# jameshball/kidney-diffusion

Hardware: AMD Instinct MI355X
Metric: denoising-steps/sec (64->256 SR UNet, bs16) (higher is better)
Workload: dtype f32

## Files before the change

include/kd_engine.h:

```cpp
#ifndef KD_ENGINE_H
#define KD_ENGINE_H

#include <stddef.h>
#include <stdint.h>

#ifdef __cplusplus
extern "C" {
#endif

#define KD_MAX_LEVELS 8

const char* kd_last_error(void);
#define KD_ENGINE_ABI_VERSION 2
int kd_version(void);
const char* kd_build_id(void);

typedef struct kd_unet_config {
  int dim;
  int num_levels;
  int dim_mults[KD_MAX_LEVELS];
  int num_resnet_blocks[KD_MAX_LEVELS];
  int layer_attns[KD_MAX_LEVELS];
  int layer_cross_attns[KD_MAX_LEVELS];
  int cond_dim;
// ... 214 lines not shown
int kd_conv3x3_winograd_nhwc(const float* d_x, const float* d_w_oihw, const float* d_bias, float* d_y,
                             int B, int H, int W, int Cin, int Cout, void* stream);
int kd_conv3x3_winograd4_nhwc(const float* d_x, const float* d_w_oihw, const float* d_bias, const float* d_res,
                              float* d_y, int B, int H, int W, int Cin, int Cout, int G, float eps,
                              float* d_out_stats, int gemm_bf16x3, void* stream);
int kd_gemm_bf16x3(const float* d_a, const float* d_b, float* d_c, int G, int M, int N, int K, int a_planes, void* stream);
int kd_linear_bf16x3(const float* d_x, int ldx, const float* d_w, const float* d_bias, const float* d_res, int ldres,
                     const float* d_gate_src, int ldgs, const float* d_gate, int hw, float* d_y, int ldy, int M, int N, int K,
                     int act, int pixshuf_wo, double* d_seg, void* stream);
int kd_linear_bf16x3_seg_rows(int M, int N, int K);
int kd_downsample_bf16x3(const float* d_x, int ldx, const float* d_w, const float* d_bias, float* d_y, int B, int H, int W, int C,
                         int O, double* d_seg, void* stream);
int kd_gn_conv3x3_winograd_fused_nhwc(const float* d_x, const float* d_gamma, const float* d_beta,
                                      const float* d_scale_shift, const float* d_w_oihw,
                                      const float* d_bias, const float* d_res, float* d_y, int B, int H,
                                      int W, int Cin, int Cout, int G, float eps, float* d_out_stats,
                                      int ldx, void* stream);

int kd_linear_skinny(const float* d_x, int ldx, const float* d_w, const float* d_bias, float* d_y, int ldy, int M, int K,
                     int N, int in_act, int act, void* stream);
int kd_global_context_gate(const float* d_x, int B, int HW, int C, const float* d_wk, const float* d_bk, const float* d_w0,
                           const float* d_b0, int hid, const float* d_w2, const float* d_b2, float* d_gate, float* d_pooled,
                           int path, void* stream);
int kd_gate_add_nhwc(const float* d_a, const float* d_gate, const float* d_r, int ldr, float* d_y, int ldy, double* d_seg,
                     int B, int HW, int C, void* stream);
int kd_gate_add_chunks(int B, int HW);
int kd_linattn_chunk_tokens(void);
int kd_linattn_dwconv_nhwc(const float* d_x, const float* d_wq, const float* d_wk, const float* d_wv, float* d_y,
                           float* d_part, int B, int H, int W, int heads, void* stream);
int kd_linattn_context(const float* d_k, const float* d_v, int ld, const float* d_part, int HW, const float* d_ck,
                       const float* d_cv, int ldc, int m, const float* d_null_k, const float* d_null_v, float* d_ctx, int B,
                       int heads, void* stream);
int kd_linattn_apply(const float* d_q, int ldq, const float* d_ctx, float* d_out, int ldo, int B, int N, int heads,
                     float scale, int silu, void* stream);
int kd_gn_fold_seg(const double* d_seg0, int nseg0, int nchunk0, float scale0, float ab_mul0, const double* d_seg1, int nseg1,
                   int nchunk1, float scale1, float ab_mul1, const float* d_gamma, const float* d_beta,
                   const float* d_scale_shift, int ld_ss, float* d_ab, float* d_stats, int B, int HW, int C, int G, float eps,
                   void* stream);
float kd_wf_ab_scale(void);
int kd_gn_conv3x3_winograd4_nhwc(const float* d_x, int ldx, const float* d_stats, const float* d_gamma, const float* d_beta,
                                 const float* d_scale_shift, int ld_ss, int skip_c0, float skip_scale, const float* d_w_oihw,
                                 const float* d_bias, const float* d_res, int ldres, float* d_y, double* d_out_seg, int B,
                                 int H, int W, int Cin, int Cout, int G, int gemm_mode, int images_per_set, void* stream);

int kd_init_conv_nchw(const float* d_x, const float* d_w3, const float* d_w7, const float* d_w15,
                      const float* d_bias, float* d_y, int B, int S, int n3, int n7, int n15, void* stream);
// ... 59 lines not shown
```

kidney-diffusion_amd/csrc/api.inc:

```
extern "C" {

const char* kd_last_error(void) { return kd::g_err.c_str(); }
int kd_version(void) { return KD_ENGINE_ABI_VERSION; }

int kd_unet_create(const kd_unet_config_t* cfg, const kd_param_t* params, int n_params, kd_unet_t** out) {
  return kd_unet_create_shared(cfg, params, n_params, nullptr, out);
}

int kd_unet_create_shared(const kd_unet_config_t* cfg, const kd_param_t* params, int n_params,
                          const kd_unet_t* share_with, kd_unet_t** out) {
  return kd_unet_create_self_cond(cfg, params, n_params, share_with, 0, out);
}

int kd_unet_create_self_cond(const kd_unet_config_t* cfg, const kd_param_t* params, int n_params,
                             const kd_unet_t* share_with, int self_cond, kd_unet_t** out) {
  kd_unet_ext_t ext;
  memset(&ext, 0, sizeof ext);
  ext.self_cond = self_cond;
  return kd_unet_create_ext(cfg, params, n_params, share_with, &ext, out);
}

int kd_unet_create_ext(const kd_unet_config_t* cfg, const kd_param_t* params, int n_params, const kd_unet_t* share_with,
                       const kd_unet_ext_t* ext, kd_unet_t** out) {
  return kd_unet_create_ext2(cfg, params, n_params, share_with, ext, nullptr, out);
// ... 680 lines not shown
}

int kd_linattn_apply(const float* d_q, int ldq, const float* d_ctx, float* d_out, int ldo, int B, int N, int heads,
                     float scale, int silu, void* stream) {
  hipStream_t s = (hipStream_t)stream;
  KD_REQUIRE(d_q && d_ctx && d_out, "kd_linattn_apply: null argument");
  return entry_finish(launch_linattn_apply(d_q, ldq, d_ctx, d_out, ldo, B, N, heads, scale, silu, s), s);
}

int kd_global_context_gate(const float* d_x, int B, int HW, int C, const float* d_wk, const float* d_bk, const float* d_w0,
                           const float* d_b0, int hid, const float* d_w2, const float* d_b2, float* d_gate, float* d_pooled,
                           int path, void* stream) {
  hipStream_t s = (hipStream_t)stream;
  KD_REQUIRE(d_x && d_wk && d_bk && d_w0 && d_b0 && d_w2 && d_b2 && d_gate, "kd_global_context_gate: null argument");
  KD_REQUIRE(B > 0 && HW > 0 && hid > 0 && C % 4 == 0 && C > 0 && C <= 2048,
             "kd_global_context_gate needs B, HW, hid > 0 and C % 4 == 0, C <= 2048");
  KD_REQUIRE(path >= 0 && path <= 2, "kd_global_context_gate: path 0 (the plan's choice), 1 (pool + two linears), 2 (fused)");
  const bool fused_ok = gca_gate_fused_ok(C, hid) && (((uintptr_t)d_w0 | (uintptr_t)d_w2) & 15) == 0;
  KD_REQUIRE(path != 2 || fused_ok, "kd_global_context_gate: the fused gate needs C <= 512, hid <= 256, 16-byte aligned weights");
  const bool fused = path == 2 || (path == 0 && gca_gate_fused_ok(C, hid) && B > 1);
  KD_REQUIRE(!(fused && d_pooled), "kd_global_context_gate: the fused gate does not leave the pooled vector");
  EntryBufs bufs;
  float *scratch = nullptr, *pooled = d_pooled, *hidden = nullptr;
  if (bufs.get((void**)&scratch, gca_scratch_floats(B, HW, C) * sizeof(float))) return 1;
  if (fused) return entry_finish(launch_gca_gate(d_x, d_wk, d_bk, scratch, d_w0, d_b0, hid, d_w2, d_b2, d_gate, B, HW, C, s), s);
  if (!pooled && bufs.get((void**)&pooled, (size_t)B * C * sizeof(float))) return 1;
  if (bufs.get((void**)&hidden, (size_t)B * hid * sizeof(float))) return 1;
  int rc = launch_gca_pool(d_x, d_wk, d_bk, nullptr, pooled, scratch, B, HW, C, s);
  if (!rc) rc = launch_linear_skinny(pooled, C, d_w0, d_b0, hidden, hid, B, C, hid, ACT_NONE, ACT_SILU, s);
  if (!rc) rc = launch_linear_skinny(hidden, hid, d_w2, d_b2, d_gate, C, B, hid, C, ACT_NONE, ACT_SIGMOID, s);
  return entry_finish(rc, s);
}

int kd_gate_add_chunks(int B, int HW) { return B > 0 && HW > 0 ? gate_add_chunks(B, HW) : 0; }

int kd_gate_add_nhwc(const float* d_a, const float* d_gate, const float* d_r, int ldr, float* d_y, int ldy, double* d_seg,
                     int B, int HW, int C, void* stream) {
  hipStream_t s = (hipStream_t)stream;
  if (ldr <= 0) ldr = C;
  if (ldy <= 0) ldy = C;
  KD_REQUIRE(d_a && d_r && d_y, "kd_gate_add_nhwc: null argument");
  KD_REQUIRE(B > 0 && HW > 0 && C > 0 && C % 4 == 0 && ldr >= C && ldy >= C && ldr % 4 == 0 && ldy % 4 == 0,
             "kd_gate_add_nhwc needs C % 4 == 0 and row strides >= C, multiples of 4");
  KD_REQUIRE((((uintptr_t)d_a | (uintptr_t)d_gate | (uintptr_t)d_r | (uintptr_t)d_y) & 15) == 0,
             "kd_gate_add_nhwc: 16-byte aligned maps and gate");
  KD_REQUIRE(!d_seg || C % 16 == 0, "kd_gate_add_nhwc: segment partials need C % 16 == 0");
  return entry_finish(launch_gate_add(d_a, d_gate, d_r, ldr, d_y, ldy, d_seg, B, HW, C, s), s);
}

float kd_wf_ab_scale(void) { return WF_AB_SCALE; }

int kd_gn_fold_seg(const double* d_seg0, int nseg0, int nchunk0, float scale0, float ab_mul0, const double* d_seg1, int nseg1,
                   int nchunk1, float scale1, float ab_mul1, const float* d_gamma, const float* d_beta,
                   const float* d_scale_shift, int ld_ss, float* d_ab, float* d_stats, int B, int HW, int C, int G, float eps,
// ... 389 lines not shown
```

kidney-diffusion_amd/csrc/common.h:

```cpp
#pragma once
#include <hip/hip_runtime.h>
#include <stdint.h>
#include <stdio.h>
#include <algorithm>
#include <string>

#ifdef KD_EXPERIMENT
#include "../../scratch/experiment_switch.h"
#else
constexpr int kd_switch(const char*, int dflt) { return dflt; }
#endif

namespace kd {

void set_error(const std::string& msg);

#define KD_HIP_CHECK(expr)                                                               \
  do {                                                                                   \
    hipError_t _e = (expr);                                                              \
    if (_e != hipSuccess) {                                                              \
      ::kd::set_error(std::string(#expr) + " failed: " + hipGetErrorString(_e) + " at " + \
                      __FILE__ + ":" + std::to_string(__LINE__));                        \
      return 1;                                                                          \
    }                                                                                    \
// ... 160 lines not shown
int launch_copy_rows(const float* src, int64_t src_bstride, int ld_src, float* dst, int64_t dst_bstride,
                     int ld_dst, int rows, int C, int B, hipStream_t s);
int launch_bcast_row(const float* src, float* dst, int64_t dst_bstride, int C, int B, hipStream_t s);

struct KVSeg {
  const float* k;
  const float* v;
  int ld;
  int n;
};
int launch_attention(const float* q, int ldq, const float* null_k, const float* null_v, KVSeg s0, KVSeg s1,
                     float* out, int ldo, int B, int Nq, int H, int Hkv, int D, float scale, hipStream_t s);
int attention_key_tile(int D);
int launch_linear_gemv(const float* x, const float* w, const float* bias, float* y, int K, int N, int in_act, int act,
                       hipStream_t s);
int launch_linear_skinny(const float* x, int ldx, const float* w, const float* bias, float* y, int ldy, int M,
                         int K, int N, int in_act, int act, hipStream_t s);
int launch_linear_skinny_valu(const float* x, int ldx, const float* w, const float* bias, float* y, int ldy, int M,
                              int K, int N, int in_act, int act, hipStream_t s);
int launch_gca_pool(const float* x, const float* wk, const float* bk, float* logits, float* pooled,
                    float* scratch, int B, int HW, int C, hipStream_t s);
size_t gca_scratch_floats(int B, int HW, int C);
bool gca_gate_fused_ok(int C, int hid);
int launch_gca_gate(const float* x, const float* wk, const float* bk, float* scratch, const float* w0, const float* b0, int hid,
                    const float* w2, const float* b2, float* gate, int B, int HW, int C, hipStream_t s);
int launch_sinu_emb(const float* t, const float* w, float* out, int B, int half, hipStream_t s);

bool init_conv_fused_ok(int S, int n3, int n7, int n15, int np);
size_t init_conv_weight_floats(int n3, int n7, int n15, int np);
int launch_init_conv_pack(const float* w3, const float* w7, const float* w15, float* out, int n3, int n7, int n15, int Itot,
                          int c0, int np, hipStream_t s);
int launch_init_conv(const float* x_nchw, const float* sc_nchw, int cx, int np, const float* wp, const float* bias, const float* res,
                     float* y, int ldy, double* seg, int B, int S, int n3, int n7, int n15, hipStream_t s);
bool init_plain_ok(int S, int n, int k, int np);
size_t init_plain_weight_floats(int n, int k, int np);
int launch_init_plain_pack(const float* w_oihw, float* out, int n, int Itot, int c0, int np, int k, hipStream_t s);
int launch_init_plain(const float* x_nchw, const float* sc_nchw, int cx, int np, const float* wp, const float* bias, const float* res,
                      float* y, int ldy, double* seg, int B, int S, int n, int k, hipStream_t s);

constexpr int LA_CHUNK = 64;
int linattn_chunks(int HW);
int linattn_splits(int B, int heads, int HW);
size_t linattn_ws_floats(int B, int heads, int HW);
int launch_linattn_pack_dw(const float* wq, const float* wk, const float* wv, float* dst, int inner, hipStream_t s);
int launch_linattn_dwconv(const float* x, const float* w, float* y, float* part, int B, int H, int W, int inner,
                          hipStream_t s);
// ... 97 lines not shown
```

kidney-diffusion_amd/csrc/engine.hip:

```cpp
#include <stdlib.h>
#include <string.h>

#include <algorithm>
#include <cstddef>
#include <functional>
#include <map>
#include <memory>
#include <stdexcept>
#include <string>
#include <type_traits>
#include <unordered_map>
#include <unordered_set>
#include <vector>

#include "../../include/kd_engine.h"
#include "common.h"

namespace kd {

static thread_local std::string g_err;
void set_error(const std::string& msg) { g_err = msg; }

#define KD_THROW_IF(expr)                                          \
  do {                                                             \
// ... 988 lines not shown
    free(proj);
    T h1 = linear(h0, P(f + ".1.weight", (int64_t)hidden * dim), nullptr, hidden, gelu_late ? ACT_NONE : ACT_GELU);
    free(h0);
    T h2 = layernorm(h1, P(f + ".3.g", hidden), nullptr, nullptr, gelu_late ? ACT_GELU : ACT_NONE, nullptr, nullptr, false,
                     linear_is_x3(h1, dim, &x1, dst) ? 1 : 0);
    free(h1);
    T y = linear(h2, P(f + ".4.weight", (int64_t)dim * hidden), nullptr, dim, ACT_NONE, &x1, dst);
    free(h2);
    free(x1);
    return y;
  }

  T gca(const T& h, const std::string& pre) {
    int C = h.C, hid = std::max(3, C / 2);
    const float* wk = P(pre + ".to_k.weight", C);
    const float* bk = P(pre + ".to_k.bias", 1);
    const float* w0 = P(pre + ".net.0.weight", (int64_t)hid * C);
    const float* b0 = P(pre + ".net.0.bias", hid);
    const float* w2 = P(pre + ".net.2.weight", (int64_t)C * hid);
    const float* b2 = P(pre + ".net.2.bias", C);
    int Bx = h.B, HW = h.HW();
    const Ref hr = at(h);
    if (gca_gate_fused_ok(C, hid) && h.B > 1 && kd_switch("KD_GCA_FUSED", 1)) {
      T scratch = alloc_bytes(gca_scratch_floats(h.B, h.HW(), C) * sizeof(float));
      T gate = alloc(h.B, 1, 1, C);
      const Ref sr = at(scratch), gr = at(gate);
      emit([=](hipStream_t s) {
        return launch_gca_gate(hr.f(), wk, bk, sr.f(), w0, b0, hid, w2, b2, gr.f(), Bx, HW, C, s);
      }, "gca_gate HW" + std::to_string(HW) + " C" + std::to_string(C));
      u->macs += (int64_t)Bx * HW * C * 2 + (int64_t)Bx * C * hid * 2;
      free(scratch);
      return gate;
    }
    T logits = alloc(h.B, h.H, h.W, 1);
    T pooled = alloc(h.B, 1, 1, C);
    T scratch = alloc_bytes(gca_scratch_floats(h.B, h.HW(), C) * sizeof(float));
    const Ref lr = at(logits), pr = at(pooled), sr = at(scratch);
    emit([=](hipStream_t s) {
      return launch_gca_pool(hr.f(), wk, bk, lr.f(), pr.f(), sr.f(), Bx, HW, C, s);
    }, "gca_pool HW" + std::to_string(HW) + " C" + std::to_string(C));
    u->macs += (int64_t)Bx * HW * C * 2;
    free(logits);
    free(scratch);
    T hidden = alloc(h.B, 1, 1, hid);
    skinny(at(pooled), C, w0, b0, at(hidden), hid, h.B, C, hid, ACT_NONE, ACT_SILU);
    free(pooled);
    T gate = alloc(h.B, 1, 1, C);
// ... 610 lines not shown
```

kidney-diffusion_amd/csrc/kernels_small.hip:

```cpp
#include "common.h"

namespace kd {

typedef float f32x16 __attribute__((ext_vector_type(16)));
typedef float f32x4 __attribute__((ext_vector_type(4)));

__device__ __forceinline__ float act_s(float v, int act) {
  if (act == ACT_SILU) return v / (1.0f + expf(-v));
  if (act == ACT_GELU) return 0.5f * v * (1.0f + erff(v * 0.70710678118654752440f));
  if (act == ACT_SIGMOID) return 1.0f / (1.0f + expf(-v));
  return v;
}
__device__ __forceinline__ float wave_sum(float v) {
#pragma unroll
  for (int off = 32; off > 0; off >>= 1) v += __shfl_xor(v, off, 64);
  return v;
}

constexpr int SKM_UNROLL = 8;

template <int KW>
__global__ __launch_bounds__(64 * KW) void linear_skinny_mfma_kernel(const float* __restrict__ x, int ldx,
                                                                    const float* __restrict__ w,
                                                                    const float* __restrict__ bias,
// ... 73 lines not shown
  KD_REQUIRE(M > 0 && N > 0 && K > 0, "skinny linear: empty");
  const bool mfma_ok = (K & 3) == 0 && (ldx & 3) == 0 && (((uintptr_t)x) & 15) == 0 && (((uintptr_t)w) & 15) == 0;
  if (!mfma_ok) return launch_linear_skinny_valu(x, ldx, w, bias, y, ldy, M, K, N, in_act, act, s);
  if (M == 1 && K <= 16384) return launch_linear_gemv(x, w, bias, y, K, N, in_act, act, s);
  dim3 grid((N + 31) / 32, (M + 31) / 32);
  if (K >= 512)
    hipLaunchKernelGGL(linear_skinny_mfma_kernel<4>, grid, dim3(256), 0, s, x, ldx, w, bias, y, ldy, M, K, N, in_act, act);
  else
    hipLaunchKernelGGL(linear_skinny_mfma_kernel<1>, grid, dim3(64), 0, s, x, ldx, w, bias, y, ldy, M, K, N, in_act, act);
  KD_HIP_CHECK(hipGetLastError());
  return 0;
}

constexpr int GCA_ROWS = 256;
static inline int gca_rows(int HW, int B) {
  int r = GCA_ROWS;
  while ((HW + r - 1) / r > 1024) r *= 2;
  while (r > 32 && (int64_t)((HW + r - 1) / r) * B < 1024 && (HW + r / 2 - 1) / (r / 2) <= 1024) r /= 2;
  return r;
}
constexpr int GCA_MAXT = 8;
constexpr int GCA_U = 4;

template <int T, int RPW>
__global__ __launch_bounds__(256) void gca_partial_kernel(const float* __restrict__ x, const float* __restrict__ wk,
                                                          const float* __restrict__ bk, float* __restrict__ part,
                                                          int HW, int C, int rows) {
  extern __shared__ float sm[];
  const int b = blockIdx.y, chunk = blockIdx.x, nchunks = gridDim.x;
  const int lane = threadIdx.x & 63, wave = threadIdx.x >> 6;
  constexpr int LPR = 64 / RPW;
  const int sub = RPW == 2 ? (lane >> 5) : 0;
  const int li = RPW == 2 ? (lane & 31) : lane;
  const int C4 = C >> 2;
  const int p0 = chunk * rows, p1 = min(HW, p0 + rows);
  f32x4 wv[T], acc[T];
  const f32x4 z = {0.f, 0.f, 0.f, 0.f};
#pragma unroll
  for (int t = 0; t < T; ++t) {
    int c4 = li + LPR * t;
    wv[t] = c4 < C4 ? *(const f32x4*)(wk + c4 * 4) : z;
    acc[t] = z;
  }
  const float bias = bk[0];
  float mrun = -INFINITY, lrun = 0.f;
  const int stride = 4 * RPW;
  for (int pb = p0 + wave * RPW + sub; pb < p1; pb += stride * GCA_U) {
    f32x4 xv[GCA_U][T];
#pragma unroll
    for (int u = 0; u < GCA_U; ++u) {
// ... 39 lines not shown
    mrun = mn;
  }
  float* sacc = sm;
  float* sml = sm + 4 * C;
  if (lane == 0) {
    sml[wave * 2] = mrun;
    sml[wave * 2 + 1] = lrun;
  }
  if (sub == 0) {
#pragma unroll
    for (int t = 0; t < T; ++t) {
      int c4 = li + LPR * t;
      if (c4 < C4) *(f32x4*)(sacc + wave * C + c4 * 4) = acc[t];
    }
  }
  __syncthreads();
  float mb = fmaxf(fmaxf(sml[0], sml[2]), fmaxf(sml[4], sml[6]));
  float sc[4], lb = 0.f;
#pragma unroll
  for (int wv_ = 0; wv_ < 4; ++wv_) {
    sc[wv_] = sml[wv_ * 2] == -INFINITY ? 0.f : expf(sml[wv_ * 2] - mb);
    lb += sml[wv_ * 2 + 1] * sc[wv_];
  }
  float* out = part + ((int64_t)b * nchunks + chunk) * (C + 2);
  for (int c = threadIdx.x; c < C; c += 256)
    out[2 + c] = (sacc[c] * sc[0] + sacc[C + c] * sc[1]) + (sacc[2 * C + c] * sc[2] + sacc[3 * C + c] * sc[3]);
  if (threadIdx.x == 0) {
    out[0] = mb;
    out[1] = lb;
  }
}

__global__ __launch_bounds__(256) void gca_combine_kernel(const float* __restrict__ part, float* __restrict__ pooled,
                                                          int nchunks, int C) {
  __shared__ float se[1024];
  __shared__ float red[8];
  __shared__ float sacc[16][16];
  const int b = blockIdx.x, lane = threadIdx.x & 63, wave = threadIdx.x >> 6;
  const int cl = threadIdx.x & 15, sub = threadIdx.x >> 4;
  const int c = blockIdx.y * 16 + cl;
  const float* pb = part + (int64_t)b * nchunks * (C + 2);
  float m = -INFINITY;
  for (int i = threadIdx.x; i < nchunks; i += 256) m = fmaxf(m, pb[(int64_t)i * (C + 2)]);
#pragma unroll
  for (int off = 32; off > 0; off >>= 1) m = fmaxf(m, __shfl_xor(m, off, 64));
  if (lane == 0) red[wave] = m;
  __syncthreads();
  const float mg = fmaxf(fmaxf(red[0], red[1]), fmaxf(red[2], red[3]));
  float l = 0.f;
  for (int i = threadIdx.x; i < nchunks; i += 256) {
    float e = expf(pb[(int64_t)i * (C + 2)] - mg);
    se[i] = e;
    l += pb[(int64_t)i * (C + 2) + 1] * e;
  }
  l = wave_sum(l);
  if (lane == 0) red[4 + wave] = l;
  __syncthreads();
  const float inv = 1.0f / ((red[4] + red[5]) + (red[6] + red[7]));
  float s = 0.f;
  if (c < C)
    for (int i = sub; i < nchunks; i += 16) s += pb[(int64_t)i * (C + 2) + 2 + c] * se[i];
  sacc[sub][cl] = s;
  __syncthreads();
  if (sub == 0 && c < C) {
    float t = 0.f;
#pragma unroll
    for (int k = 0; k < 16; ++k) t += sacc[k][cl];
    pooled[(int64_t)b * C + c] = t * inv;
  }
}

constexpr int GCAG_MAXC = 512;
__global__ __launch_bounds__(256) void gca_gate_kernel(const float* __restrict__ part, int nchunks, int C,
                                                       const float* __restrict__ w0, const float* __restrict__ b0, int hid,
                                                       const float* __restrict__ w2, const float* __restrict__ b2,
                                                       float* __restrict__ gate) {
  __shared__ float se[1024];
  __shared__ float red[8];
  __shared__ __attribute__((aligned(16))) float pooled[GCAG_MAXC];
  __shared__ __attribute__((aligned(16))) float hidden[GCAG_MAXC / 2];
  const int b = blockIdx.x, lane = threadIdx.x & 63, wave = threadIdx.x >> 6;
  const float* pb = part + (int64_t)b * nchunks * (C + 2);
  float m = -INFINITY;
  for (int i = threadIdx.x; i < nchunks; i += 256) m = fmaxf(m, pb[(int64_t)i * (C + 2)]);
#pragma unroll
  for (int off = 32; off > 0; off >>= 1) m = fmaxf(m, __shfl_xor(m, off, 64));
  if (lane == 0) red[wave] = m;
  __syncthreads();
  const float mg = fmaxf(fmaxf(red[0], red[1]), fmaxf(red[2], red[3]));
  float l = 0.f;
  for (int i = threadIdx.x; i < nchunks; i += 256) {
    const float e = expf(pb[(int64_t)i * (C + 2)] - mg);
    se[i] = e;
    l += pb[(int64_t)i * (C + 2) + 1] * e;
  }
  l = wave_sum(l);
  if (lane == 0) red[4 + wave] = l;
  __syncthreads();
  const float inv = 1.0f / ((red[4] + red[5]) + (red[6] + red[7]));
  for (int c = threadIdx.x; c < C; c += 256) {
    float s0 = 0.f, s1 = 0.f, s2 = 0.f, s3 = 0.f;
    int i = 0;
    for (; i + 3 < nchunks; i += 4) {
      s0 = fmaf(pb[(int64_t)i * (C + 2) + 2 + c], se[i], s0);
      s1 = fmaf(pb[(int64_t)(i + 1) * (C + 2) + 2 + c], se[i + 1], s1);
      s2 = fmaf(pb[(int64_t)(i + 2) * (C + 2) + 2 + c], se[i + 2], s2);
      s3 = fmaf(pb[(int64_t)(i + 3) * (C + 2) + 2 + c], se[i + 3], s3);
    }
    for (; i < nchunks; ++i) s0 = fmaf(pb[(int64_t)i * (C + 2) + 2 + c], se[i], s0);
    pooled[c] = ((s0 + s1) + (s2 + s3)) * inv;
  }
  __syncthreads();
  typedef float f32x4g __attribute__((ext_vector_type(4)));
  for (int h = threadIdx.x; h < hid; h += 256) {
    const f32x4g* wr = (const f32x4g*)(w0 + (int64_t)h * C);
    float a0 = 0.f, a1 = 0.f, a2 = 0.f, a3 = 0.f;
    for (int c4 = 0; c4 < C / 4; ++c4) {
      const f32x4g wv = wr[c4], pv = *(const f32x4g*)(pooled + 4 * c4);
      a0 = fmaf(wv[0], pv[0], a0);
      a1 = fmaf(wv[1], pv[1], a1);
      a2 = fmaf(wv[2], pv[2], a2);
      a3 = fmaf(wv[3], pv[3], a3);
    }
    const float v = ((a0 + a1) + (a2 + a3)) + b0[h];
    hidden[h] = v / (1.0f + expf(-v));
  }
  __syncthreads();
  for (int n = threadIdx.x; n < C; n += 256) {
    const float* wr = w2 + (int64_t)n * hid;
    float a0 = 0.f, a1 = 0.f;
    int h = 0;
    if ((hid & 3) == 0) {
      float a2 = 0.f, a3 = 0.f;
      for (; h < hid; h += 4) {
        const f32x4g wv = *(const f32x4g*)(wr + h), hv = *(const f32x4g*)(hidden + h);
        a0 = fmaf(wv[0], hv[0], a0);
        a1 = fmaf(wv[1], hv[1], a1);
        a2 = fmaf(wv[2], hv[2], a2);
        a3 = fmaf(wv[3], hv[3], a3);
      }
      a0 += a2;
      a1 += a3;
    } else {
      for (; h < hid; ++h) a0 = fmaf(wr[h], hidden[h], a0);
    }
    const float v = (a0 + a1) + b2[n];
    gate[(int64_t)b * C + n] = 1.0f / (1.0f + expf(-v));
  }
}

bool gca_gate_fused_ok(int C, int hid) {
  return C % 4 == 0 && C <= GCAG_MAXC && hid <= GCAG_MAXC / 2 && hid > 0;
}

static int launch_gca_partial(const float* x, const float* wk, const float* bk, float* scratch, int B, int HW, int C, int rows,
                              int chunks, hipStream_t s) {
  size_t smem = (size_t)(4 * C + 8) * sizeof(float);
  const int C4 = C / 4;
  dim3 grid(chunks, B), blk(256);
  if (C4 == 32) hipLaunchKernelGGL((gca_partial_kernel<1, 2>), grid, blk, smem, s, x, wk, bk, scratch, HW, C, rows);
  else if (C4 <= 64) hipLaunchKernelGGL((gca_partial_kernel<1, 1>), grid, blk, smem, s, x, wk, bk, scratch, HW, C, rows);
  else if (C4 <= 128) hipLaunchKernelGGL((gca_partial_kernel<2, 1>), grid, blk, smem, s, x, wk, bk, scratch, HW, C, rows);
  else if (C4 <= 256) hipLaunchKernelGGL((gca_partial_kernel<4, 1>), grid, blk, smem, s, x, wk, bk, scratch, HW, C, rows);
  else hipLaunchKernelGGL((gca_partial_kernel<8, 1>), grid, blk, smem, s, x, wk, bk, scratch, HW, C, rows);
  KD_HIP_CHECK(hipGetLastError());
  return 0;
}

int launch_gca_gate(const float* x, const float* wk, const float* bk, float* scratch, const float* w0, const float* b0, int hid,
                    const float* w2, const float* b2, float* gate, int B, int HW, int C, hipStream_t s) {
  KD_REQUIRE(gca_gate_fused_ok(C, hid), "fused GlobalContext gate needs C % 4 == 0, C <= 512, hidden <= 256");
  KD_REQUIRE((((uintptr_t)w0 | (uintptr_t)w2) & 15) == 0, "fused GlobalContext gate: 16-byte aligned weights");
  const int rows = gca_rows(HW, B), chunks = (HW + rows - 1) / rows;
  if (launch_gca_partial(x, wk, bk, scratch, B, HW, C, rows, chunks, s)) return 1;
  hipLaunchKernelGGL(gca_gate_kernel, dim3(B), dim3(256), 0, s, scratch, chunks, C, w0, b0, hid, w2, b2, gate);
  KD_HIP_CHECK(hipGetLastError());
  return 0;
}

size_t gca_scratch_floats(int B, int HW, int C) {
  int rows = gca_rows(HW, B), chunks = (HW + rows - 1) / rows;
  return (size_t)B * chunks * (C + 2);
}

int launch_gca_pool(const float* x, const float* wk, const float* bk, float* , float* pooled,
                    float* scratch, int B, int HW, int C, hipStream_t s) {
  KD_REQUIRE(C % 4 == 0 && C <= 64 * 4 * GCA_MAXT, "gca needs C % 4 == 0 and C <= 2048");
  const int rows = gca_rows(HW, B), chunks = (HW + rows - 1) / rows;
  if (launch_gca_partial(x, wk, bk, scratch, B, HW, C, rows, chunks, s)) return 1;
  hipLaunchKernelGGL(gca_combine_kernel, dim3(B, (C + 15) / 16), dim3(256), 0, s, scratch, pooled, chunks, C);
  KD_HIP_CHECK(hipGetLastError());
  return 0;
}

}
```

kidney-diffusion_amd/imagen_pytorch/_engine.py:

```python
from __future__ import annotations

import ctypes as C
import os
from pathlib import Path

KD_MAX_LEVELS = 8

_LIB_PATH = Path(__file__).resolve().parent.parent / "lib" / "libkd_engine.so"


class EngineUnavailable(RuntimeError):
    pass


class EngineError(RuntimeError):
    pass


class kd_unet_config_t(C.Structure):
    _fields_ = [
        ("dim", C.c_int),
        ("num_levels", C.c_int),
        ("dim_mults", C.c_int * KD_MAX_LEVELS),
        ("num_resnet_blocks", C.c_int * KD_MAX_LEVELS),
# ... 159 lines not shown
    "kd_solver_sample_steps": (C.c_int, [C.c_void_p, C.POINTER(kd_solver_schedule_t), C.POINTER(kd_sample_args_t), C.c_void_p,
                                         C.c_int, C.c_int, C.c_void_p]),
    "kd_conv2d_nhwc": (C.c_int, [C.c_void_p] * 4 + [C.c_int] * 10 + [C.c_void_p]),
    "kd_upsample_nearest_conv3x3_nhwc": (C.c_int, [C.c_void_p] * 4 + [C.c_int] * 7 + [C.c_void_p]),
    "kd_upsample_nearest_gn_conv3x3_nhwc": (C.c_int, [C.c_void_p, C.c_int] + [C.c_void_p] * 4 + [C.c_int] * 8 + [C.c_void_p]),
    "kd_conv3x3_winograd_nhwc": (C.c_int, [C.c_void_p] * 4 + [C.c_int] * 5 + [C.c_void_p]),
    "kd_conv3x3_winograd4_nhwc": (C.c_int, [C.c_void_p] * 5 + [C.c_int] * 6 + [C.c_float, C.c_void_p, C.c_int, C.c_void_p]),
    "kd_gemm_bf16x3": (C.c_int, [C.c_void_p] * 3 + [C.c_int] * 5 + [C.c_void_p]),
    "kd_linear_bf16x3": (C.c_int, [C.c_void_p, C.c_int, C.c_void_p, C.c_void_p, C.c_void_p, C.c_int, C.c_void_p, C.c_int,
                                   C.c_void_p, C.c_int, C.c_void_p, C.c_int, C.c_int, C.c_int, C.c_int, C.c_int, C.c_int, C.c_void_p,
                                   C.c_void_p]),
    "kd_linear_bf16x3_seg_rows": (C.c_int, [C.c_int, C.c_int, C.c_int]),
    "kd_downsample_bf16x3": (C.c_int, [C.c_void_p, C.c_int, C.c_void_p, C.c_void_p, C.c_void_p] + [C.c_int] * 5 + [C.c_void_p, C.c_void_p]),
    "kd_gn_conv3x3_winograd_fused_nhwc": (C.c_int, [C.c_void_p] * 8 + [C.c_int] * 6 + [C.c_float, C.c_void_p, C.c_int, C.c_void_p]),
    "kd_linattn_chunk_tokens": (C.c_int, []),
    "kd_linattn_dwconv_nhwc": (C.c_int, [C.c_void_p] * 6 + [C.c_int] * 4 + [C.c_void_p]),
    "kd_linattn_context": (C.c_int, [C.c_void_p, C.c_void_p, C.c_int, C.c_void_p, C.c_int, C.c_void_p, C.c_void_p, C.c_int,
                                     C.c_int, C.c_void_p, C.c_void_p, C.c_void_p, C.c_int, C.c_int, C.c_void_p]),
    "kd_linattn_apply": (C.c_int, [C.c_void_p, C.c_int, C.c_void_p, C.c_void_p, C.c_int, C.c_int, C.c_int, C.c_int,
                                   C.c_float, C.c_int, C.c_void_p]),
    "kd_linear_skinny": (C.c_int, [C.c_void_p, C.c_int, C.c_void_p, C.c_void_p, C.c_void_p] + [C.c_int] * 6 + [C.c_void_p]),
    "kd_global_context_gate": (C.c_int, [C.c_void_p] + [C.c_int] * 3 + [C.c_void_p] * 4 + [C.c_int] + [C.c_void_p] * 4 +
                               [C.c_int, C.c_void_p]),
    "kd_gate_add_nhwc": (C.c_int, [C.c_void_p] * 3 + [C.c_int, C.c_void_p, C.c_int, C.c_void_p] + [C.c_int] * 3 + [C.c_void_p]),
    "kd_gate_add_chunks": (C.c_int, [C.c_int, C.c_int]),
    "kd_gn_fold_seg": (C.c_int, [C.c_void_p, C.c_int, C.c_int, C.c_float, C.c_float, C.c_void_p, C.c_int, C.c_int, C.c_float,
                                 C.c_float] + [C.c_void_p] * 3 + [C.c_int] + [C.c_void_p] * 2 + [C.c_int] * 4 +
                       [C.c_float, C.c_void_p]),
    "kd_wf_ab_scale": (C.c_float, []),
    "kd_gn_conv3x3_winograd4_nhwc": (C.c_int, [C.c_void_p, C.c_int] + [C.c_void_p] * 4 + [C.c_int, C.c_int, C.c_float] +
                                     [C.c_void_p] * 3 + [C.c_int] + [C.c_void_p] * 2 + [C.c_int] * 8 + [C.c_void_p]),
    "kd_init_conv_nchw": (C.c_int, [C.c_void_p] * 6 + [C.c_int] * 5 + [C.c_void_p]),
    "kd_init_conv_planes_nchw": (C.c_int, [C.c_void_p] * 5 + [C.c_int] * 2 + [C.c_void_p] * 3 + [C.c_int] * 6 +
                                 [C.POINTER(C.c_float), C.c_void_p]),
    "kd_init_conv_planes_c_nchw": (C.c_int, [C.c_void_p] * 5 + [C.c_int] * 2 + [C.c_void_p] * 3 + [C.c_int] * 6 +
                                   [C.POINTER(C.c_float), C.c_int, C.c_void_p]),
    "kd_final_conv_nchw": (C.c_int, [C.c_void_p] * 5 + [C.c_int] * 5 + [C.c_void_p]),
    "kd_final_conv_k_nchw": (C.c_int, [C.c_void_p] * 5 + [C.c_int] * 6 + [C.c_void_p]),
    "kd_init_conv_plain_nchw": (C.c_int, [C.c_void_p] * 3 + [C.c_int] * 2 + [C.c_void_p] * 3 + [C.c_int] + [C.c_void_p] +
                                [C.c_int] * 6 + [C.POINTER(C.c_float), C.c_void_p]),
    "kd_groupnorm_silu_nhwc": (C.c_int, [C.c_void_p] * 5 + [C.c_int] * 4 + [C.c_float, C.c_void_p]),
    "kd_layernorm": (C.c_int, [C.c_void_p] * 4 + [C.c_int, C.c_int, C.c_float, C.c_void_p]),
    "kd_layernorm_ex": (C.c_int, [C.c_void_p] * 5 + [C.c_int, C.c_int, C.c_float, C.c_int, C.c_void_p, C.c_void_p, C.c_void_p]),
    "kd_layernorm_linear_bf16x3": (C.c_int, [C.c_void_p] * 3 + [C.c_int, C.c_int, C.c_float, C.c_int] + [C.c_void_p] * 3 +
                                   [C.c_int, C.c_void_p, C.c_int, C.c_int, C.c_void_p, C.c_void_p]),
    "kd_attention_ex_d": (C.c_int, [C.c_void_p, C.c_int, C.c_void_p, C.c_void_p, C.c_void_p, C.c_int, C.c_int, C.c_void_p,
# ... 120 lines not shown
```

Measured before the change: 40.65.

## Fold first gate linear into GlobalContext partial pass and parallelize chunk combine

When hid*C is small, the per-chunk partial kernel now applies the first linear layer (w0) to its local softmax-weighted pooled vector and stores hid-wide partials instead of C-wide ones. This is valid because the combine step is linear. The gate kernel then combines fewer values per chunk, spreads the chunk reduction across sub-groups of threads when the width is at most 256, and caches the chunk max and sum in registers. Scratch sizing gains a new helper, and a chunk-count query is exported. The trade is redundant w0 matvecs in every chunk block in exchange for less scratch traffic and a shorter serial tail in the single-block-per-batch gate kernel.

```diff
diff --git a/include/kd_engine.h b/include/kd_engine.h
--- a/include/kd_engine.h
+++ b/include/kd_engine.h
@@ -260,6 +260,7 @@
 int kd_global_context_gate(const float* d_x, int B, int HW, int C, const float* d_wk, const float* d_bk, const float* d_w0,
                            const float* d_b0, int hid, const float* d_w2, const float* d_b2, float* d_gate, float* d_pooled,
                            int path, void* stream);
+int kd_global_context_gate_chunks(int B, int HW, int C, int hid);
 int kd_gate_add_nhwc(const float* d_a, const float* d_gate, const float* d_r, int ldr, float* d_y, int ldy, double* d_seg,
                      int B, int HW, int C, void* stream);
 int kd_gate_add_chunks(int B, int HW);
diff --git a/kidney-diffusion_amd/csrc/api.inc b/kidney-diffusion_amd/csrc/api.inc
--- a/kidney-diffusion_amd/csrc/api.inc
+++ b/kidney-diffusion_amd/csrc/api.inc
@@ -726,7 +726,8 @@
   KD_REQUIRE(!(fused && d_pooled), "kd_global_context_gate: the fused gate does not leave the pooled vector");
   EntryBufs bufs;
   float *scratch = nullptr, *pooled = d_pooled, *hidden = nullptr;
-  if (bufs.get((void**)&scratch, gca_scratch_floats(B, HW, C) * sizeof(float))) return 1;
+  const size_t scratch_floats = fused ? gca_gate_scratch_floats(B, HW, C, hid) : gca_scratch_floats(B, HW, C);
+  if (bufs.get((void**)&scratch, scratch_floats * sizeof(float))) return 1;
   if (fused) return entry_finish(launch_gca_gate(d_x, d_wk, d_bk, scratch, d_w0, d_b0, hid, d_w2, d_b2, d_gate, B, HW, C, s), s);
   if (!pooled && bufs.get((void**)&pooled, (size_t)B * C * sizeof(float))) return 1;
   if (bufs.get((void**)&hidden, (size_t)B * hid * sizeof(float))) return 1;
@@ -734,6 +735,10 @@
   if (!rc) rc = launch_linear_skinny(pooled, C, d_w0, d_b0, hidden, hid, B, C, hid, ACT_NONE, ACT_SILU, s);
   if (!rc) rc = launch_linear_skinny(hidden, hid, d_w2, d_b2, d_gate, C, B, hid, C, ACT_NONE, ACT_SIGMOID, s);
   return entry_finish(rc, s);
+}
+
+int kd_global_context_gate_chunks(int B, int HW, int C, int hid) {
+  return B > 0 && HW > 0 && gca_gate_fused_ok(C, hid) ? gca_gate_chunks(B, HW, C, hid) : 0;
 }
 
 int kd_gate_add_chunks(int B, int HW) { return B > 0 && HW > 0 ? gate_add_chunks(B, HW) : 0; }
diff --git a/kidney-diffusion_amd/csrc/common.h b/kidney-diffusion_amd/csrc/common.h
--- a/kidney-diffusion_amd/csrc/common.h
+++ b/kidney-diffusion_amd/csrc/common.h
@@ -206,6 +206,8 @@
                     float* scratch, int B, int HW, int C, hipStream_t s);
 size_t gca_scratch_floats(int B, int HW, int C);
 bool gca_gate_fused_ok(int C, int hid);
+size_t gca_gate_scratch_floats(int B, int HW, int C, int hid);
+int gca_gate_chunks(int B, int HW, int C, int hid);
 int launch_gca_gate(const float* x, const float* wk, const float* bk, float* scratch, const float* w0, const float* b0, int hid,
                     const float* w2, const float* b2, float* gate, int B, int HW, int C, hipStream_t s);
 int launch_sinu_emb(const float* t, const float* w, float* out, int B, int half, hipStream_t s);
diff --git a/kidney-diffusion_amd/csrc/engine.hip b/kidney-diffusion_amd/csrc/engine.hip
--- a/kidney-diffusion_amd/csrc/engine.hip
+++ b/kidney-diffusion_amd/csrc/engine.hip
@@ -1034,7 +1034,7 @@
     int Bx = h.B, HW = h.HW();
     const Ref hr = at(h);
     if (gca_gate_fused_ok(C, hid) && h.B > 1 && kd_switch("KD_GCA_FUSED", 1)) {
-      T scratch = alloc_bytes(gca_scratch_floats(h.B, h.HW(), C) * sizeof(float));
+      T scratch = alloc_bytes(gca_gate_scratch_floats(h.B, h.HW(), C, hid) * sizeof(float));
       T gate = alloc(h.B, 1, 1, C);
       const Ref sr = at(scratch), gr = at(gate);
       emit([=](hipStream_t s) {
diff --git a/kidney-diffusion_amd/csrc/kernels_small.hip b/kidney-diffusion_amd/csrc/kernels_small.hip
--- a/kidney-diffusion_amd/csrc/kernels_small.hip
+++ b/kidney-diffusion_amd/csrc/kernels_small.hip
@@ -119,10 +119,10 @@
 constexpr int GCA_MAXT = 8;
 constexpr int GCA_U = 4;
 
-template <int T, int RPW>
+template <int T, int RPW, bool FC>
 __global__ __launch_bounds__(256) void gca_partial_kernel(const float* __restrict__ x, const float* __restrict__ wk,
                                                           const float* __restrict__ bk, float* __restrict__ part,
-                                                          int HW, int C, int rows) {
+                                                          int HW, int C, int rows, const float* __restrict__ w0, int hid) {
   extern __shared__ float sm[];
   const int b = blockIdx.y, chunk = blockIdx.x, nchunks = gridDim.x;
   const int lane = threadIdx.x & 63, wave = threadIdx.x >> 6;
@@ -208,12 +208,47 @@
     sc[wv_] = sml[wv_ * 2] == -INFINITY ? 0.f : expf(sml[wv_ * 2] - mb);
     lb += sml[wv_ * 2 + 1] * sc[wv_];
   }
-  float* out = part + ((int64_t)b * nchunks + chunk) * (C + 2);
-  for (int c = threadIdx.x; c < C; c += 256)
-    out[2 + c] = (sacc[c] * sc[0] + sacc[C + c] * sc[1]) + (sacc[2 * C + c] * sc[2] + sacc[3 * C + c] * sc[3]);
+  float* out = part + ((int64_t)b * nchunks + chunk) * ((FC ? hid : C) + 2);
   if (threadIdx.x == 0) {
     out[0] = mb;
     out[1] = lb;
+  }
+  if (!FC) {
+    for (int c = threadIdx.x; c < C; c += 256)
+      out[2 + c] = (sacc[c] * sc[0] + sacc[C + c] * sc[1]) + (sacc[2 * C + c] * sc[2] + sacc[3 * C + c] * sc[3]);
+    return;
+  }
+  for (int c = threadIdx.x; c < C; c += 256)
+    sacc[c] = (sacc[c] * sc[0] + sacc[C + c] * sc[1]) + (sacc[2 * C + c] * sc[2] + sacc[3 * C + c] * sc[3]);
+  __syncthreads();
+#pragma unroll
+  for (int t = 0; t < T; ++t) {
+    int c4 = li + LPR * t;
+    acc[t] = c4 < C4 ? *(const f32x4*)(sacc + c4 * 4) : z;
+  }
+  for (int hb = wave * RPW; hb < hid; hb += stride * GCA_U) {
+    f32x4 xv[GCA_U][T];
+#pragma unroll
+    for (int u = 0; u < GCA_U; ++u) {
+      const int h = hb + sub + u * stride;
+      const float* wr = w0 + (int64_t)(h < hid ? h : 0) * C;
+#pragma unroll
+      for (int t = 0; t < T; ++t) {
+        int c4 = li + LPR * t;
+        xv[u][t] = c4 < C4 ? *(const f32x4*)(wr + c4 * 4) : z;
+      }
+    }
+#pragma unroll
+    for (int u = 0; u < GCA_U; ++u) {
+      float d = 0.f;
+#pragma unroll
+      for (int t = 0; t < T; ++t)
+        d += (xv[u][t][0] * acc[t][0] + xv[u][t][1] * acc[t][1]) + (xv[u][t][2] * acc[t][2] + xv[u][t][3] * acc[t][3]);
+#pragma unroll
+      for (int off = LPR / 2; off > 0; off >>= 1) d += __shfl_xor(d, off, 64);
+      const int h = hb + sub + u * stride;
+      if (li == 0 && h < hid) out[2 + h] = d;
+    }
   }
 }
 
@@ -257,7 +292,31 @@
 }
 
 constexpr int GCAG_MAXC = 512;
-__global__ __launch_bounds__(256) void gca_gate_kernel(const float* __restrict__ part, int nchunks, int C,
+constexpr int GCAG_D = 8;
+__device__ __forceinline__ void gca_row_dot(const float* __restrict__ wr, const float* v, int n4, float (&a)[4]) {
+  typedef float f32x4g __attribute__((ext_vector_type(4)));
+  const f32x4g* w4 = (const f32x4g*)wr;
+  const f32x4g* v4 = (const f32x4g*)v;
+  int k = 0;
+  for (; k + GCAG_D <= n4; k += GCAG_D) {
+    f32x4g wv[GCAG_D];
+#pragma unroll
+    for (int u = 0; u < GCAG_D; ++u) wv[u] = w4[k + u];
+#pragma unroll
+    for (int u = 0; u < GCAG_D; ++u) {
+      const f32x4g pv = v4[k + u];
+#pragma unroll
+      for (int e = 0; e < 4; ++e) a[e] = fmaf(wv[u][e], pv[e], a[e]);
+    }
+  }
+  for (; k < n4; ++k) {
+    const f32x4g wv = w4[k], pv = v4[k];
+#pragma unroll
+    for (int e = 0; e < 4; ++e) a[e] = fmaf(wv[e], pv[e], a[e]);
+  }
+}
+
+__global__ __launch_bounds__(256) void gca_gate_kernel(const float* __restrict__ part, int nchunks, int C, bool fc1,
                                                        const float* __restrict__ w0, const float* __restrict__ b0, int hid,
                                                        const float* __restrict__ w2, const float* __restrict__ b2,
                                                        float* __restrict__ gate) {
@@ -265,72 +324,97 @@
   __shared__ float red[8];
   __shared__ __attribute__((aligned(16))) float pooled[GCAG_MAXC];
   __shared__ __attribute__((aligned(16))) float hidden[GCAG_MAXC / 2];
+  __shared__ float ssub[256];
   const int b = blockIdx.x, lane = threadIdx.x & 63, wave = threadIdx.x >> 6;
-  const float* pb = part + (int64_t)b * nchunks * (C + 2);
-  float m = -INFINITY;
-  for (int i = threadIdx.x; i < nchunks; i += 256) m = fmaxf(m, pb[(int64_t)i * (C + 2)]);
+  const int W = fc1 ? hid : C, R = W + 2;
+  const float* pb = part + (int64_t)b * nchunks * R;
+  float mi[4], li[4], m = -INFINITY;
+#pragma unroll
+  for (int k = 0; k < 4; ++k) {
+    const int i = threadIdx.x + 256 * k;
+    mi[k] = i < nchunks ? pb[(int64_t)i * R] : -INFINITY;
+    li[k] = i < nchunks ? pb[(int64_t)i * R + 1] : 0.f;
+    m = fmaxf(m, mi[k]);
+  }
 #pragma unroll
   for (int off = 32; off > 0; off >>= 1) m = fmaxf(m, __shfl_xor(m, off, 64));
   if (lane == 0) red[wave] = m;
   __syncthreads();
   const float mg = fmaxf(fmaxf(red[0], red[1]), fmaxf(red[2], red[3]));
   float l = 0.f;
-  for (int i = threadIdx.x; i < nchunks; i += 256) {
-    const float e = expf(pb[(int64_t)i * (C + 2)] - mg);
-    se[i] = e;
-    l += pb[(int64_t)i * (C + 2) + 1] * e;
+#pragma unroll
+  for (int k = 0; k < 4; ++k) {
+    const int i = threadIdx.x + 256 * k;
+    if (i < nchunks) {
+      const float e = expf(mi[k] - mg);
+      se[i] = e;
+      l += li[k] * e;
+    }
   }
   l = wave_sum(l);
   if (lane == 0) red[4 + wave] = l;
   __syncthreads();
   const float inv = 1.0f / ((red[4] + red[5]) + (red[6] + red[7]));
-  for (int c = threadIdx.x; c < C; c += 256) {
+  float* vec = fc1 ? hidden : pooled;
+  if (W <= 256) {
+    int WP = 1;
+    while (WP < W) WP <<= 1;
+    const int NS = 256 / WP, cl = threadIdx.x & (WP - 1), sub = threadIdx.x / WP;
     float s0 = 0.f, s1 = 0.f, s2 = 0.f, s3 = 0.f;
-    int i = 0;
-    for (; i + 3 < nchunks; i += 4) {
-      s0 = fmaf(pb[(int64_t)i * (C + 2) + 2 + c], se[i], s0);
-      s1 = fmaf(pb[(int64_t)(i + 1) * (C + 2) + 2 + c], se[i + 1], s1);
-      s2 = fmaf(pb[(int64_t)(i + 2) * (C + 2) + 2 + c], se[i + 2], s2);
-      s3 = fmaf(pb[(int64_t)(i + 3) * (C + 2) + 2 + c], se[i + 3], s3);
-    }
-    for (; i < nchunks; ++i) s0 = fmaf(pb[(int64_t)i * (C + 2) + 2 + c], se[i], s0);
-    pooled[c] = ((s0 + s1) + (s2 + s3)) * inv;
-  }
-  __syncthreads();
-  typedef float f32x4g __attribute__((ext_vector_type(4)));
-  for (int h = threadIdx.x; h < hid; h += 256) {
-    const f32x4g* wr = (const f32x4g*)(w0 + (int64_t)h * C);
-    float a0 = 0.f, a1 = 0.f, a2 = 0.f, a3 = 0.f;
-    for (int c4 = 0; c4 < C / 4; ++c4) {
-      const f32x4g wv = wr[c4], pv = *(const f32x4g*)(pooled + 4 * c4);
-      a0 = fmaf(wv[0], pv[0], a0);
-      a1 = fmaf(wv[1], pv[1], a1);
-      a2 = fmaf(wv[2], pv[2], a2);
-      a3 = fmaf(wv[3], pv[3], a3);
-    }
-    const float v = ((a0 + a1) + (a2 + a3)) + b0[h];
+    if (cl < W) {
+      const float* pc = pb + 2 + cl;
+      int i = sub;
+      for (; i + 3 * NS < nchunks; i += 4 * NS) {
+        s0 = fmaf(pc[(int64_t)i * R], se[i], s0);
+        s1 = fmaf(pc[(int64_t)(i + NS) * R], se[i + NS], s1);
+        s2 = fmaf(pc[(int64_t)(i + 2 * NS) * R], se[i + 2 * NS], s2);
+        s3 = fmaf(pc[(int64_t)(i + 3 * NS) * R], se[i + 3 * NS], s3);
+      }
+      for (; i < nchunks; i += NS) s0 = fmaf(pc[(int64_t)i * R], se[i], s0);
+    }
+    ssub[threadIdx.x] = (s0 + s1) + (s2 + s3);
+    __syncthreads();
+    if (threadIdx.x < W) {
+      float t = 0.f;
+      for (int k = 0; k < NS; ++k) t += ssub[k * WP + threadIdx.x];
+      t *= inv;
+      if (fc1) {
+        t += b0[threadIdx.x];
+        t = t / (1.0f + expf(-t));
+      }
+      vec[threadIdx.x] = t;
+    }
+  } else {
+    for (int c = threadIdx.x; c < W; c += 256) {
+      float s0 = 0.f, s1 = 0.f, s2 = 0.f, s3 = 0.f;
+      int i = 0;
+      for (; i + 3 < nchunks; i += 4) {
+        s0 = fmaf(pb[(int64_t)i * R + 2 + c], se[i], s0);
+        s1 = fmaf(pb[(int64_t)(i + 1) * R + 2 + c], se[i + 1], s1);
+        s2 = fmaf(pb[(int64_t)(i + 2) * R + 2 + c], se[i + 2], s2);
+        s3 = fmaf(pb[(int64_t)(i + 3) * R + 2 + c], se[i + 3], s3);
+      }
+      for (; i < nchunks; ++i) s0 = fmaf(pb[(int64_t)i * R + 2 + c], se[i], s0);
+      pooled[c] = ((s0 + s1) + (s2 + s3)) * inv;
+    }
+  }
+  __syncthreads();
+  for (int h = threadIdx.x; !fc1 && h < hid; h += 256) {
+    float a[4] = {0.f, 0.f, 0.f, 0.f};
+    gca_row_dot(w0 + (int64_t)h * C, pooled, C / 4, a);
+    const float v = ((a[0] + a[1]) + (a[2] + a[3])) + b0[h];
     hidden[h] = v / (1.0f + expf(-v));
   }
   __syncthreads();
   for (int n = threadIdx.x; n < C; n += 256) {
     const float* wr = w2 + (int64_t)n * hid;
-    float a0 = 0.f, a1 = 0.f;
-    int h = 0;
+    float a[4] = {0.f, 0.f, 0.f, 0.f};
     if ((hid & 3) == 0) {
-      float a2 = 0.f, a3 = 0.f;
-      for (; h < hid; h += 4) {
-        const f32x4g wv = *(const f32x4g*)(wr + h), hv = *(const f32x4g*)(hidden + h);
-        a0 = fmaf(wv[0], hv[0], a0);
-        a1 = fmaf(wv[1], hv[1], a1);
-        a2 = fmaf(wv[2], hv[2], a2);
-        a3 = fmaf(wv[3], hv[3], a3);
-      }
-      a0 += a2;
-      a1 += a3;
+      gca_row_dot(wr, hidden, hid / 4, a);
     } else {
-      for (; h < hid; ++h) a0 = fmaf(wr[h], hidden[h], a0);
-    }
-    const float v = (a0 + a1) + b2[n];
+      for (int h = 0; h < hid; ++h) a[0] = fmaf(wr[h], hidden[h], a[0]);
+    }
+    const float v = ((a[0] + a[2]) + (a[1] + a[3])) + b2[n];
     gate[(int64_t)b * C + n] = 1.0f / (1.0f + expf(-v));
   }
 }
@@ -339,30 +423,55 @@
   return C % 4 == 0 && C <= GCAG_MAXC && hid <= GCAG_MAXC / 2 && hid > 0;
 }
 
-static int launch_gca_partial(const float* x, const float* wk, const float* bk, float* scratch, int B, int HW, int C, int rows,
-                              int chunks, hipStream_t s) {
+template <bool FC>
+static int launch_gca_partial_t(const float* x, const float* wk, const float* bk, float* scratch, int B, int HW, int C,
+                                int rows, int chunks, const float* w0, int hid, hipStream_t s) {
   size_t smem = (size_t)(4 * C + 8) * sizeof(float);
   const int C4 = C / 4;
   dim3 grid(chunks, B), blk(256);
-  if (C4 == 32) hipLaunchKernelGGL((gca_partial_kernel<1, 2>), grid, blk, smem, s, x, wk, bk, scratch, HW, C, rows);
-  else if (C4 <= 64) hipLaunchKernelGGL((gca_partial_kernel<1, 1>), grid, blk, smem, s, x, wk, bk, scratch, HW, C, rows);
-  else if (C4 <= 128) hipLaunchKernelGGL((gca_partial_kernel<2, 1>), grid, blk, smem, s, x, wk, bk, scratch, HW, C, rows);
-  else if (C4 <= 256) hipLaunchKernelGGL((gca_partial_kernel<4, 1>), grid, blk, smem, s, x, wk, bk, scratch, HW, C, rows);
-  else hipLaunchKernelGGL((gca_partial_kernel<8, 1>), grid, blk, smem, s, x, wk, bk, scratch, HW, C, rows);
+#define KD_GCA_PARTIAL(T, RPW) \
+  hipLaunchKernelGGL((gca_partial_kernel<T, RPW, FC>), grid, blk, smem, s, x, wk, bk, scratch, HW, C, rows, w0, hid)
+  if (C4 == 32) KD_GCA_PARTIAL(1, 2);
+  else if (C4 <= 64) KD_GCA_PARTIAL(1, 1);
+  else if (C4 <= 128) KD_GCA_PARTIAL(2, 1);
+  else if (C4 <= 256) KD_GCA_PARTIAL(4, 1);
+  else KD_GCA_PARTIAL(8, 1);
+#undef KD_GCA_PARTIAL
   KD_HIP_CHECK(hipGetLastError());
   return 0;
+}
+static int launch_gca_partial(const float* x, const float* wk, const float* bk, float* scratch, int B, int HW, int C, int rows,
+                              int chunks, const float* w0, int hid, hipStream_t s) {
+  return w0 ? launch_gca_partial_t<true>(x, wk, bk, scratch, B, HW, C, rows, chunks, w0, hid, s)
+            : launch_gca_partial_t<false>(x, wk, bk, scratch, B, HW, C, rows, chunks, nullptr, 0, s);
+}
+
+struct GcaGateForm { int rows, chunks; bool fc1; };
+static GcaGateForm gca_gate_form(int B, int HW, int C, int hid) {
+  GcaGateForm f;
+  f.rows = gca_rows(HW, B);
+  f.chunks = (HW + f.rows - 1) / f.rows;
+  f.fc1 = (int64_t)hid * C <= 8192;
+  return f;
 }
 
 int launch_gca_gate(const float* x, const float* wk, const float* bk, float* scratch, const float* w0, const float* b0, int hid,
                     const float* w2, const float* b2, float* gate, int B, int HW, int C, hipStream_t s) {
   KD_REQUIRE(gca_gate_fused_ok(C, hid), "fused GlobalContext gate needs C % 4 == 0, C <= 512, hidden <= 256");
   KD_REQUIRE((((uintptr_t)w0 | (uintptr_t)w2) & 15) == 0, "fused GlobalContext gate: 16-byte aligned weights");
-  const int rows = gca_rows(HW, B), chunks = (HW + rows - 1) / rows;
-  if (launch_gca_partial(x, wk, bk, scratch, B, HW, C, rows, chunks, s)) return 1;
-  hipLaunchKernelGGL(gca_gate_kernel, dim3(B), dim3(256), 0, s, scratch, chunks, C, w0, b0, hid, w2, b2, gate);
+  const GcaGateForm f = gca_gate_form(B, HW, C, hid);
+  if (launch_gca_partial(x, wk, bk, scratch, B, HW, C, f.rows, f.chunks, f.fc1 ? w0 : nullptr, hid, s)) return 1;
+  hipLaunchKernelGGL(gca_gate_kernel, dim3(B), dim3(256), 0, s, scratch, f.chunks, C, f.fc1, w0, b0, hid, w2, b2, gate);
   KD_HIP_CHECK(hipGetLastError());
   return 0;
 }
+
+size_t gca_gate_scratch_floats(int B, int HW, int C, int hid) {
+  const GcaGateForm f = gca_gate_form(B, HW, C, hid);
+  return (size_t)B * f.chunks * ((f.fc1 ? hid : C) + 2);
+}
+
+int gca_gate_chunks(int B, int HW, int C, int hid) { return gca_gate_form(B, HW, C, hid).chunks; }
 
 size_t gca_scratch_floats(int B, int HW, int C) {
   int rows = gca_rows(HW, B), chunks = (HW + rows - 1) / rows;
@@ -373,7 +482,7 @@
                     float* scratch, int B, int HW, int C, hipStream_t s) {
   KD_REQUIRE(C % 4 == 0 && C <= 64 * 4 * GCA_MAXT, "gca needs C % 4 == 0 and C <= 2048");
   const int rows = gca_rows(HW, B), chunks = (HW + rows - 1) / rows;
-  if (launch_gca_partial(x, wk, bk, scratch, B, HW, C, rows, chunks, s)) return 1;
+  if (launch_gca_partial(x, wk, bk, scratch, B, HW, C, rows, chunks, nullptr, 0, s)) return 1;
   hipLaunchKernelGGL(gca_combine_kernel, dim3(B, (C + 15) / 16), dim3(256), 0, s, scratch, pooled, chunks, C);
   KD_HIP_CHECK(hipGetLastError());
   return 0;
diff --git a/kidney-diffusion_amd/imagen_pytorch/_engine.py b/kidney-diffusion_amd/imagen_pytorch/_engine.py
--- a/kidney-diffusion_amd/imagen_pytorch/_engine.py
+++ b/kidney-diffusion_amd/imagen_pytorch/_engine.py
@@ -205,6 +205,7 @@
     "kd_linear_skinny": (C.c_int, [C.c_void_p, C.c_int, C.c_void_p, C.c_void_p, C.c_void_p] + [C.c_int] * 6 + [C.c_void_p]),
     "kd_global_context_gate": (C.c_int, [C.c_void_p] + [C.c_int] * 3 + [C.c_void_p] * 4 + [C.c_int] + [C.c_void_p] * 4 +
                                [C.c_int, C.c_void_p]),
+    "kd_global_context_gate_chunks": (C.c_int, [C.c_int] * 4),
     "kd_gate_add_nhwc": (C.c_int, [C.c_void_p] * 3 + [C.c_int, C.c_void_p, C.c_int, C.c_void_p] + [C.c_int] * 3 + [C.c_void_p]),
     "kd_gate_add_chunks": (C.c_int, [C.c_int, C.c_int]),
     "kd_gn_fold_seg": (C.c_int, [C.c_void_p, C.c_int, C.c_int, C.c_float, C.c_float, C.c_void_p, C.c_int, C.c_int, C.c_float,
```

New measurement: 40.77, median of 6. Within noise of the previous version (+0.3%).
